# Iasonaspg/GPU-Randomized-Block-Lanczos

Hardware: AMD Instinct MI355X
Metric: RBL iters/sec + time-to-k=20 eigenpairs, n=1e7 nnz/row=100 b=32; 1/2/4/8 GPU (higher is better)
Workload: dtype f64

## Files before the change

### gpu-randomized-block-lanczos_amd/csrc/kernels.hpp

```cpp
#pragma once
#include "rbl_common.hpp"

namespace rbl {

struct Panels {
  static constexpr int kMax = 2;
  const double* ptr[kMax] = {nullptr, nullptr};
  int count = 0;
  int w = 0;
};
struct PanelRun {
  const double* base = nullptr;
  const float* base32 = nullptr;
  int64_t stride = 0;
  int count = 0;
  int w = 0;
};

constexpr int64_t kCsrPad = 256;
constexpr int64_t kRowPad = 16;
constexpr int64_t kRowPad32 = 32;

struct CsrDev {
  int64_t nrows = 0;
// ... 253 lines not shown
                 hipStream_t s);
int reduce_scratch_splits(int splits);
void reduce_slab_many(double* slab, int splits, int64_t len, double* out, hipStream_t s);
void tsmm(int64_t nrows, const PanelRun& X, const double* C, int ldc, const Panels& Y,
          double alpha, double beta, const int* skip, hipStream_t s, double* xslab = nullptr,
          int* xgrid = nullptr);

constexpr int kCompressMaxCols = 512;
bool basis_compress_fast(const PanelRun& X, int p);
bool basis_compress(int64_t nrows, const PanelRun& X, const double* S_dev, int p, hipStream_t s,
                    bool generic = false);

bool gram44_ok(int64_t nrows, int nW, int w, int xcount, int xw);
int gram44_splits(int64_t nrows, int nW, int w = 32);
void gram44_partial(int64_t nrows, const PanelRun& W, const Panels& X, double* slab, int splits,
                    const int* skip, hipStream_t s);
bool tsmm44_ok(int xw, int ky, int yw);
void tsmm44_f32x(int64_t nrows, const PanelRun& X, const double* C, int ldc, const Panels& Y,
                 double alpha, double beta, hipStream_t s);
int tsmm44_xg_grid(int64_t nrows);
void tsmm44(int64_t nrows, const PanelRun& X, const double* C, int ldc, const Panels& Y,
            double alpha, double beta, const int* skip, hipStream_t s, double* xslab = nullptr,
            int* xgrid = nullptr);

int gram32_splits(int64_t nrows);
void gram32_partial(int64_t nrows, const float* Wb, int64_t wstride, int nW, int w, const float* X0,
                    const float* X1, int xcount, double* slab, int splits, hipStream_t s);
void tsmm32(int64_t nrows, const float* Xb, int64_t xstride, int nX, int w, const double* C, int ldc,
            float* Y0, float* Y1, int ycount, float alpha, float beta, hipStream_t s);
void cvt_f32_to_f64(const float* src, double* dst, int64_t n, hipStream_t s);
void cvt_f64_to_f32(const double* src, float* dst, int64_t n, hipStream_t s);

void chol_step(const double* G, int b, int64_t nglobal, int mode, double* R, double* Rinv,
               double* Rtot, int* need3, int* status, const int* skip, hipStream_t s,
               double* scratch);
void copy_small(const double* src, double* dst, int64_t len, hipStream_t s, const int* skip = nullptr);
void cloc_rinv(double* C, const double* Rinv, int b, const int* skip, hipStream_t s);
void cloc_rinv2(double* C, const double* R1inv, const double* R2inv, int b, hipStream_t s);
void cloc_gate(const double* R, const double* Rinv, int b, const int* need3, double tau, int* gate,
               hipStream_t s);
void cloc_sub(double* G, const double* D, int nW, int b, hipStream_t s);
void transpose_small(const double* src, double* dst, int b, hipStream_t s);
void stash_step(const double* Ai, const double* Rtot, double* Bprev, int* flags, double* stash,
                int b, hipStream_t s);

struct RmatParams {
  int64_t n = 0;
  int scale = 0;
  int64_t edges = 0;
  double a = 0.57, b = 0.19, c = 0.19;
  uint64_t seed = 0;
  bool relabel = false;
  Scatter perm;
};
constexpr uint64_t kRelabelK = 0x52454C4142454C31ull;
void rmat_degree(const RmatParams& p, int32_t* deg, hipStream_t s);
int rmat_local_csr(const RmatParams& p, int64_t r0, int64_t r1, int64_t max_keys, int nplant,
                   const double* plant_dev, int64_t* rowptr_dev, int32_t** col_dev,
                   double** val_dev, int64_t* nnz_out, hipStream_t s);
void col_footprint(const int32_t* col, int64_t nnz, const int64_t* bounds_dev, int P,
                   unsigned long long* lo, unsigned long long* hi, hipStream_t s);

void circ_count(int64_t n, int64_t width, double p, uint64_t seed, int64_t r0, int64_t r1,
// ... 22 lines not shown
```

### gpu-randomized-block-lanczos_amd/csrc/rbl_api.cpp

```cpp
#include <hip/hip_runtime.h>
#include <rocprofiler-sdk-roctx/roctx.h>

#include <algorithm>
#include <cstdlib>
#include <chrono>
#include <cmath>
#include <cstdio>
#include <cstring>
#include <string>
#include <thread>
#include <vector>

#include "../../include/rbl_hip.h"
#include "comm.hpp"
#include "kernels.hpp"

using namespace rbl;

namespace rbl::api {

template <class T>
struct DevBuf {
  T* p = nullptr;
  DevBuf() = default;
// ... 148 lines not shown
  DevBuf<double> d_U;
  DevBuf<double> d_T;
  DevBuf<double> d_qext;
  DevBuf<double> d_sendbuf;
  DevBuf<double> d_pushbuf;
  DevBuf<double> d_precv;
  DevBuf<double> d_slab;
  DevBuf<double> d_C;
  DevBuf<double> d_small;
  DevBuf<int> d_flags;
  PinBuf<double> h_pin;
  PinBuf<double> h_hist;
  DevBuf<double> d_stash;
  DevBuf<double> d_lock;
  DevBuf<double> d_arrow_W;
  DevBuf<double> d_tr_S;
  DevBuf<double> d_filt[3];
  DevBuf<double> d_rv;
  DevBuf<double> d_rw;
};

struct CtxBufs {
  PinBuf<char> h_d2h[2];
};

}

struct rbl_ctx : rbl::api::MatrixBufs, rbl::api::RunBufs, rbl::api::CtxBufs {
  int device = 0;
  hipStream_t stream = nullptr;
  int nranks = 1, rank = 0;
  rbl::Comm* comm = nullptr;
  std::string err;

  int64_t n = 0, r0 = 0, r1 = 0, nloc = 0, nnz = 0;
  int64_t panel_nblk = 0;
  int panel_rpg = 4;
  int panel_ch = 48;
  bool panel_auto = false;
  int64_t panel_span = 0;
  int bt_ng = 0;
  int64_t seg_ntasks = 0, seg_nlong = 0;
  int seg_ntiers = 0;
  bool seg_split = false;
  bool ghost = false;
  int64_t n_ghost = 0, n_send = 0;
// ... 61 lines not shown
  double* dv_pin = nullptr;
  double* dv_hist = nullptr;
  bool flags_clean = false;
  int fetched = 1;
  bool have_bprev = false;
  int nlock = 0, lock_cap = 0;
  int arrow_kb = 0;
  size_t arrow_W_cap = 0, tr_S_cap = 0;
  int filt_deg = 0;
  double filt_lo = 0.0, filt_hi = 0.0, filt_ref = 0.0;
  int filt_cols = 0;
  std::vector<double> ser_mu;
  double ser_lo = 0.0, ser_hi = 0.0;
  int ritz_k = 0;

  int timers = 0;
  int reorth_order = 0;
  int spmm_variant = 0;
  int fuse = 7;
  int cloc_step = 0;
  bool cloc_final = false;
  bool cloc_derive = true;
  int cloc_src = 0;
  bool plan_all_resident = false;
  std::vector<int> step_flags;
  double stage_ms[RBL_NUM_STAGES] = {0};
  int64_t comm_stats[RBL_COMM_NSTATS] = {0};
  int64_t comm_host_ns[2] = {0, 0};
  double comm_dev_ms[2] = {0.0, 0.0};
  int64_t path_stats[RBL_PATH_NSTATS] = {0};
  struct Mark { int stage; hipEvent_t a, b; int parent = -1; };
  std::vector<Mark> marks;
  struct OpenStage { int stage; hipStream_t st; };
  std::vector<OpenStage> open_stages;
  std::vector<hipEvent_t> ev_pool;
  size_t ev_used = 0;
};

using namespace rbl::api;

namespace {

const char* kStageNames[RBL_NUM_STAGES] = {"AQ", "3-term", "qr", "part reorth", "loc reorth",
                                           "Ritz vectors", "comm", "spill wait"};

int fail(rbl_ctx* c, int code, const std::string& msg) {
// ... 1303 lines not shown
  const int d = (int)mu.size() - 1;
  const double c = 0.5 * (ctx->ser_lo + ctx->ser_hi), e = 0.5 * (ctx->ser_hi - ctx->ser_lo);
  const double* t1 = X;
  const double* t2 = nullptr;
  const int64_t len = ctx->nloc * b;
  for (int j = 1; j <= d; ++j) {
    double* tj = F[j % 3];
    const int st = apply_A(ctx, t1, 0, b, tj, nullptr, nullptr, nullptr);
    if (st < 0) return st;
    const double al = (j == 1 ? 1.0 : 2.0) / e;
    cheb_series_term(len, tj, t1, t2, al, -al * c, mu[j], mu[0], tj, out, j == 1, j == d, ctx->stream);
    HIPC(hipGetLastError());
    t2 = t1;
    t1 = tj;
  }
  return RBL_OK;
}

int filter_apply(rbl_ctx* ctx, const double* X, int b, double* out, const DevBuf<double> F[3]) {
  if (has_series(ctx)) return series_apply(ctx, X, b, out, F);
  return cheb_apply(ctx, X, b, out, F[0], F[1]);
}

int lock_reorth(rbl_ctx* ctx, double* X) {
  const int b = ctx->b;
  for (int j = 0; j < ctx->nlock; ++j) {
    const double* l = ctx->d_lock + (int64_t)j * ctx->nloc;
    CHK(gram(ctx, run1(l, 1), pan1(X, b), ctx->d_C, nullptr));
    CHK(tsmm_checked(ctx, run1(l, 1), ctx->d_C, b, pan1(X, b), -1.0, 1.0, nullptr));
  }
  return RBL_OK;
}

bool cloc_derive_on(const rbl_ctx* ctx) {
  return ctx->cloc_derive && ctx->basis_bits == 64 && rowgram_ok(ctx->b) && (ctx->fuse & 3) == 3 &&
         ctx->reorth_order == 0 && !spilled(ctx) && (ctx->nranks == 1 || ctx->plan_all_resident);
}

int reorth_pair(rbl_ctx* ctx, int i, int flags) {
  const int b = ctx->b;
  double* Qi = slotp(ctx, i - 1);
  double* Qm = i >= 2 ? slotp(ctx, i - 2) : nullptr;
  if ((flags & 2) && ctx->nlock > 0) {
    StageScope t(ctx, RBL_STAGE_PART_REORTH);
    if (Qm) CHK(lock_reorth(ctx, Qm));
    CHK(lock_reorth(ctx, Qi));
  }
  if ((flags & 1) && i >= 3) {
    StageScope t(ctx, RBL_STAGE_PART_REORTH);
    const int nW = i - 2;
    const int nres = std::min(nW, ctx->resident);
    const bool derive = cloc_derive_on(ctx) && b == 32 && ctx->cloc_step == i && !ctx->cloc_final &&
                        !((flags & 2) && ctx->nlock > 0) && nres == nW;
    const bool xg = (ctx->fuse & 2) && b == 32 && !derive;
    const int xg_parts = tsmm44_xg_grid(ctx->nloc);
    const bool xslab_ok = (size_t)(xg_parts + reduce_scratch_splits(xg_parts)) * b * b <= ctx->slab_elems;
    int xgrid = 0;
    auto update = [&](const PanelRun& W, bool last) -> int {
      const bool here = xg && last && xslab_ok;
      return tsmm_checked(ctx, W, ctx->d_C, 2 * b, pan2(Qi, Qm, b), -1.0, 1.0, nullptr,
                          here ? ctx->d_slab : nullptr, here ? &xgrid : nullptr);
    };
    if (ctx->reorth_order == 0) {
      PanelRun W;
      W.base = slotp(ctx, 0);
      W.stride = ctx->slot;
      W.count = nres;
      W.w = b;
      CHK(gram(ctx, W, pan2(Qi, Qm, b), ctx->d_C, nullptr));
      CHK(update(W, nres == nW));
    } else {
      for (int j = 0; j < nres; ++j) {
        const PanelRun W = run1(slotp(ctx, j), b);
        CHK(gram(ctx, W, pan2(Qi, Qm, b), ctx->d_C, nullptr));
        CHK(update(W, j == nW - 1));
      }
    }
    for (int j = nres; j < nW; ++j) {
      int st = 0;
      const double* Wj = block_dev(ctx, j, i, &st);
      if (st) return fail(ctx, st, "partial reorth: H2D of a spilled block failed");
      CHK(gram(ctx, run1(Wj, b), pan2(Qi, Qm, b), ctx->d_C, nullptr));
      CHK(update(run1(Wj, b), j == nW - 1));
    }
    if (xg) {
      if (xgrid > 0) {
        reduce_slab_many(ctx->d_slab, xgrid, (int64_t)b * b, smallp(ctx, S_CLOC), ctx->stream);
      } else if (ctx->nloc > 0) {
        const int sp = gram_splits(ctx->nloc, 1, b, b);
        gram_partial(ctx->nloc, run1(Qm, b), pan1(Qi, b), ctx->d_slab, sp, nullptr, ctx->stream);
        reduce_slab(ctx->d_slab, sp, (int64_t)b * b, smallp(ctx, S_CLOC), nullptr, ctx->stream);
      } else {
        HIPC(hipMemsetAsync(smallp(ctx, S_CLOC), 0, (size_t)b * b * sizeof(double), ctx->stream));
// ... 858 lines not shown
      if (value < 0 || value > 7 || value == 4)
        return fail(ctx, RBL_ERR_INVALID, "spmm kernel must be 0 (auto) or a kernel id 1, 2, 3, 5, 6, 7");
      ctx->spmm_variant = value == 5 ? 4 : value == 6 ? 5 : (int)value;
      return RBL_OK;
    case RBL_OPT_SPLIT_HALO: ctx->split_halo = value != 0; return RBL_OK;
    case RBL_OPT_HALO_OVERLAP: ctx->halo_overlap = value != 0; return RBL_OK;
    case RBL_OPT_HALO_PUSH:
      if (value < 0 || value > 2) return fail(ctx, RBL_ERR_INVALID, "RBL_OPT_HALO_PUSH must be 0|1|2");
      ctx->halo_push_opt = (int)value;
      return RBL_OK;
    case RBL_OPT_KEEP_CSR: ctx->keep_csr = value != 0; return RBL_OK;
    case RBL_OPT_RELABEL:
      if (value < 0 || value > 1) return fail(ctx, RBL_ERR_INVALID, "RBL_OPT_RELABEL must be 0|1");
      ctx->relabel_opt = (int)value;
      return RBL_OK;
    case RBL_OPT_FUSE:
      if (value < 0 || value > 7) return fail(ctx, RBL_ERR_INVALID, "RBL_OPT_FUSE is a 3-bit mask");
      ctx->fuse = (int)value;
      return RBL_OK;
    case RBL_OPT_CLOC_DERIVE:
      if (value < 0 || value > 1) return fail(ctx, RBL_ERR_INVALID, "RBL_OPT_CLOC_DERIVE must be 0|1");
      ctx->cloc_derive = value != 0;
      return RBL_OK;
    default: return fail(ctx, RBL_ERR_INVALID, "unknown option");
  }
}

int rbl_set_matrix_csc(rbl_ctx* ctx, int64_t n, int64_t nnz, const int64_t* colptr,
                       const int64_t* rowval, const double* nzval, int index_base) {
  if (!ctx || n < 1 || nnz < 0 || !colptr || (nnz && (!rowval || !nzval)) ||
      (index_base != 0 && index_base != 1))
    return fail(ctx, RBL_ERR_INVALID, "rbl_set_matrix_csc: bad arguments");
  if (colptr[n] - colptr[0] != nnz) return fail(ctx, RBL_ERR_INVALID, "colptr[n] != nnz");
  HIPC(hipSetDevice(ctx->device));
  std::vector<int64_t> rp(n + 1);
  for (int64_t i = 0; i <= n; ++i) rp[i] = colptr[i] - colptr[0];
  ctx->bounds.assign(ctx->nranks + 1, 0);
  rbl_plan_row_partition(n, rp.data(), ctx->nranks, ctx->bounds.data());
  const int64_t r0 = ctx->bounds[ctx->rank], r1 = ctx->bounds[ctx->rank + 1];
  return upload_csr(ctx, n, r0, r1, colptr + r0, rowval, nzval, index_base, index_base);
}

int rbl_set_matrix_csr_rows(rbl_ctx* ctx, int64_t n, int64_t row_begin, int64_t row_end,
                            const int64_t* rowptr, const int64_t* colind, const double* val,
                            int index_base) {
  if (!ctx || n < 1 || row_begin < 0 || row_end < row_begin || row_end > n || !rowptr ||
// ... 864 lines not shown
      HIPC(hipMemsetAsync(ctx->d_stage32, 0, ((size_t)nl + kRowPad32) * b * sizeof(float), ctx->stream));
      CHK(ensure_spill_stream(ctx));
    }
    HIPC(ctx->d_Qi64.alloc((nl + kRowPad) * b));
    if (!direct32_ok(ctx, b)) HIPC(ctx->d_Qm64.alloc((nl + kRowPad) * b));
  }
  HIPC(ctx->d_U.alloc((nl + kRowPad) * b));
  ctx->T_cols = b;
  HIPC(ctx->d_T.alloc(nl * b));
  if (ctx->nranks > 1) {
    CHK(ensure_qext(ctx, b, ctx->stream));
    if (ctx->ghost)
      HIPC(ctx->d_sendbuf.alloc(std::max<int64_t>(ctx->n_send, 1) * b));
  }
  const size_t slab = gram_slab_elems(ctx, b, max_blocks, basis_bits);
  ctx->slab_elems = slab;
  HIPC(ctx->d_slab.alloc(slab));
  ctx->C_elems = (size_t)std::max(1, max_blocks) * b * 2 * b;
  HIPC(ctx->d_C.alloc(ctx->C_elems));
  HIPC(ctx->d_small.alloc((size_t)S_NSMALL * b * b));
  HIPC(hipMemset(ctx->d_small, 0, (size_t)S_NSMALL * b * b * sizeof(double)));
  HIPC(ctx->d_flags.alloc(6));
  HIPC(hipMemset(ctx->d_flags, 0, 6 * sizeof(int)));
  {
#ifdef RBL_VARIANTS
    const char* e = std::getenv("RBL_STASH_COPY");
    ctx->stash_direct = !(e && std::atoi(e) == 1);
#else
    ctx->stash_direct = true;
#endif
    const unsigned hf = ctx->stash_direct ? (hipHostMallocMapped | hipHostMallocCoherent) : hipHostMallocDefault;
    HIPC(ctx->h_pin.alloc(stash_rec(b), hf));
    HIPC(ctx->h_hist.alloc((size_t)(max_blocks + 2) * stash_rec(b), hf));
    if ((size_t)ctx->nloc * b * sizeof(double) >= 4 * kD2HPiece && !d2h_direct()) {
      CHK(ensure_d2h_slots(ctx));
      CHK(ensure_ritz_stream(ctx));
    }
    if (ctx->stash_direct) {
      HIPC(hipHostGetDevicePointer(reinterpret_cast<void**>(&ctx->dv_pin), ctx->h_pin, 0));
      HIPC(hipHostGetDevicePointer(reinterpret_cast<void**>(&ctx->dv_hist), ctx->h_hist, 0));
    } else {
      HIPC(ctx->d_stash.alloc(stash_rec(b)));
    }
  }
  }
  if (ctx->push && ctx->nranks > 1 && use_ghost(ctx, b)) {
// ... 1677 lines not shown
  return RBL_OK;
}

int rbl_comm_stats(rbl_ctx* ctx, int64_t* out, int nstats, int reset) {
  if (!ctx || nstats < 0 || (nstats > 0 && !out)) return RBL_ERR_INVALID;
  for (int i = 0; i < nstats && i < RBL_COMM_NSTATS; ++i) out[i] = ctx->comm_stats[i];
  if (nstats > RBL_COMM_HALO_PUSH) out[RBL_COMM_HALO_PUSH] = ctx->push ? 1 : 0;
  if (nstats > RBL_COMM_PUSH_ROWS) out[RBL_COMM_PUSH_ROWS] = ctx->push_pred_rows;
  if (nstats > RBL_COMM_PULL_ROWS) out[RBL_COMM_PULL_ROWS] = ctx->pull_pred_rows;
  const int64_t tm[4] = {ctx->comm_host_ns[0], ctx->comm_host_ns[1],
                         (int64_t)(ctx->comm_dev_ms[0] * 1e6), (int64_t)(ctx->comm_dev_ms[1] * 1e6)};
  for (int i = RBL_COMM_PULL_ROWS + 1; i < nstats; ++i)
    out[i] = i <= RBL_COMM_EXCHANGE_DEV_NS ? tm[i - RBL_COMM_ALLREDUCE_HOST_NS] : 0;
  if (reset) {
    for (int64_t& v : ctx->comm_stats) v = 0;
    ctx->comm_host_ns[0] = ctx->comm_host_ns[1] = 0;
    ctx->comm_dev_ms[0] = ctx->comm_dev_ms[1] = 0.0;
  }
  return RBL_OK;
}

int rbl_path_stats(rbl_ctx* ctx, int64_t* out, int nstats, int reset) {
  if (!ctx || nstats < 0 || (nstats > 0 && !out)) return RBL_ERR_INVALID;
  for (int i = 0; i < nstats; ++i) out[i] = i < RBL_PATH_NSTATS ? ctx->path_stats[i] : 0;
  if (reset)
    for (int64_t& v : ctx->path_stats) v = 0;
  return RBL_OK;
}

int rbl_reset_timers(rbl_ctx* ctx) {
  if (!ctx) return RBL_ERR_INVALID;
  for (double& v : ctx->stage_ms) v = 0.0;
  return RBL_OK;
}
int rbl_synchronize(rbl_ctx* ctx) {
  if (!ctx) return RBL_ERR_INVALID;
  HIPC(hipSetDevice(ctx->device));
  HIPC(hipStreamSynchronize(ctx->stream));
  harvest_timers(ctx);
  return RBL_OK;
}

}
```

### gpu-randomized-block-lanczos_amd/csrc/reorth.hip

```cpp
#include <algorithm>
#include <cstdlib>

#include "kernels.hpp"

namespace rbl {

__device__ __forceinline__ double mfma4(double a, double b, double c) {
  return __builtin_amdgcn_mfma_f64_4x4x4f64(a, b, c, 0, 0, 0);
}
#ifndef RBL_REORTH_ABL
#define RBL_REORTH_ABL 0
#endif
#ifndef RBL_REORTH_NT
#define RBL_REORTH_NT 0
#endif
template <typename T>
__device__ __forceinline__ T ldw(const T* p) {
  if constexpr (RBL_REORTH_NT) return __builtin_nontemporal_load(p);
  return *p;
}

constexpr int kG44Waves = 4;
#ifndef RBL_G44_ROWS
#define RBL_G44_ROWS 16
// ... 756 lines not shown
      }
    }
  }
  if constexpr (XG) {
    __syncthreads();
    const int li = lane & 15;
    constexpr int G2 = YW * YW;
    double* gw = cs_raw + wave * G2;
#pragma unroll
    for (int it = 0; it < NT; ++it)
#pragma unroll
      for (int jt = 0; jt < NT; ++jt)
#pragma unroll
        for (int reg = 0; reg < 4; ++reg) gw[(16 * it + q + 4 * reg) * YW + 16 * jt + li] = gx[it][jt][reg];
    __syncthreads();
    double* out = xslab + tile * G2;
    for (int e = tid; e < G2; e += 256)
      out[e] = (cs_raw[e] + cs_raw[G2 + e]) + (cs_raw[2 * G2 + e] + cs_raw[3 * G2 + e]);
  }
  };
  tile_body(blockIdx.x);
}

bool tsmm44_ok(int xw, int ky, int yw) {
  return (xw == 16 || xw == 32) && ky >= 1 && ky <= 64 && yw % 2 == 0;
}

template <int B, int KYP, bool F32X = false>
static void launch_tsmm44(int64_t nrows, const PanelRun& X, const double* C, int ldc, int KY,
                          const Panels& Y, double alpha, double beta, const int* skip,
                          hipStream_t st) {
  const int64_t wgs = (nrows + 4 * kT44Rows - 1) / (4 * kT44Rows);
  hipLaunchKernelGGL((k_tsmm44<B, KYP, F32X>), dim3((unsigned)wgs), dim3(256), 0, st, nrows, X, C,
                     ldc, KY, Y, alpha, beta, skip);
}

void tsmm44_f32x(int64_t nrows, const PanelRun& X, const double* C, int ldc, const Panels& Y,
                 double alpha, double beta, hipStream_t st) {
  const int KY = Y.count * Y.w;
  if (X.w == 32) {
    if (KY <= 16) return launch_tsmm44<32, 16, true>(nrows, X, C, ldc, KY, Y, alpha, beta, nullptr, st);
    if (KY <= 32) return launch_tsmm44<32, 32, true>(nrows, X, C, ldc, KY, Y, alpha, beta, nullptr, st);
    return launch_tsmm44<32, 64, true>(nrows, X, C, ldc, KY, Y, alpha, beta, nullptr, st);
  }
  if (KY <= 16) return launch_tsmm44<16, 16, true>(nrows, X, C, ldc, KY, Y, alpha, beta, nullptr, st);
  if (KY <= 32) return launch_tsmm44<16, 32, true>(nrows, X, C, ldc, KY, Y, alpha, beta, nullptr, st);
// ... 72 lines not shown
```

### gpu-randomized-block-lanczos_amd/csrc/smallmat.hip

```cpp
#include <cstdlib>

#include "kernels.hpp"

namespace rbl {

constexpr int kMaxB = 64;

template <bool LDS>
struct SmallMat {
  double* p;
  int ld;
  __device__ double& operator()(int r, int c) const { return p[r * ld + c]; }
};

template <bool LDS>
__global__ __launch_bounds__(256) void k_chol(const double* __restrict__ G, int b, int64_t nglob,
                                              int mode, double* R, double* Rinv, double* Rtot,
                                              int* need3, int* status, const int* skip,
                                              double* scratch) {
  if (skip && *skip) return;
  __shared__ double Ml[LDS ? kMaxB * (kMaxB + 1) : 1];
  __shared__ double Xl[LDS ? kMaxB * (kMaxB + 1) : 1];
  __shared__ int fail;
  __shared__ double shift;
// ... 565 lines not shown
  const int c = threadIdx.x;
  double s = 0.0;
  if (c < b)
    for (int k = 0; k <= c; ++k) s += rs[k * b + c] * rs[k * b + c];
  d[c] = sqrt(s);
  __syncthreads();
  double t = 0.0;
  if (c < b)
    for (int j = 0; j <= c; ++j) t += d[j] * fabs(ri[j * b + c]);
  e[c] = t;
  __syncthreads();
  if (c == 0) {
    bool ok = need3[0] == 0;
    for (int j = 0; j < b; ++j) ok = ok && e[j] <= tau;
    gate[0] = ok;
    gate[1] = !ok;
  }
}
void cloc_gate(const double* R, const double* Rinv, int b, const int* need3, double tau, int* gate,
               hipStream_t s) {
  hipLaunchKernelGGL(k_cloc_gate, dim3(1), dim3(256), 0, s, R, Rinv, b, need3, tau, gate);
}

constexpr int kClocSubThreads = 1024;
__global__ __launch_bounds__(kClocSubThreads) void k_cloc_sub(double* __restrict__ G,
                                                              const double* __restrict__ D, int K, int b) {
  __shared__ double part[kClocSubThreads];
  const int r = blockIdx.x, ng = kClocSubThreads / b;
  const int kg = threadIdx.x / b, c = threadIdx.x % b;
  const int chunk = (K + ng - 1) / ng;
  double acc = 0.0;
  if (kg < ng) {
    const int k1 = min(K, (kg + 1) * chunk);
    for (int k = kg * chunk; k < k1; ++k) acc += D[(int64_t)k * 2 * b + b + r] * D[(int64_t)k * 2 * b + c];
  }
  part[threadIdx.x] = acc;
  __syncthreads();
  if (kg == 0) {
    double sum = part[c];
    for (int g = 1; g < ng; ++g) sum += part[g * b + c];
    G[r * b + c] -= sum;
  }
}
void cloc_sub(double* G, const double* D, int nW, int b, hipStream_t s) {
  hipLaunchKernelGGL(k_cloc_sub, dim3(b), dim3(kClocSubThreads), 0, s, G, D, nW * b, b);
}
// ... 10 lines not shown
```

### gpu-randomized-block-lanczos_amd/rbl/_lib.py

```python
from __future__ import annotations

import ctypes as C
import os

import numpy as np

_HERE = os.path.dirname(os.path.abspath(__file__))
LIB_PATH = os.environ.get("RBL_LIB") or os.path.join(_HERE, "librbl_hip.so")

RBL_OK = 0
RBL_WARN_NOT_CONVERGED = 1
RBL_WARN_QR_SHIFTED = 2
RBL_ERR_INVALID = -1
RBL_ERR_HIP = -2
RBL_ERR_OOM = -3
RBL_ERR_RCCL = -4
RBL_ERR_STATE = -5
RBL_ERR_NUMERIC = -6

RBL_MAX_BLOCK = 512

RBL_OPT_TIMERS = 0
RBL_OPT_REORTH_ORDER = 1
RBL_OPT_SPMM_KERNEL = 2
RBL_OPT_DEVICE_BLOCKS = 3
RBL_OPT_SPLIT_HALO = 4
RBL_OPT_KEEP_CSR = 5
RBL_OPT_FUSE = 6
RBL_OPT_HALO_OVERLAP = 7
RBL_OPT_RELABEL = 8
RBL_OPT_HALO_PUSH = 9
RBL_OPT_CLOC_DERIVE = 10
RBL_PATH_SPMM = 0
RBL_PATH_SPMM_LOC_FUSED = 1
RBL_PATH_LOC_SEPARATE = 2
RBL_PATH_LOC_GRAM = 3
RBL_PATH_LOCFIX_EDGES = 4
RBL_PATH_LOCFIX_REST = 5
RBL_PATH_SPMM_TWO_WAVE = 6
RBL_PATH_RITZ_PIECES = 7
RBL_PATH_CLOC_3TERM = 8
RBL_PATH_CLOC_REORTH = 9
RBL_PATH_NSTATS = 10
RBL_BUILD_VARIANTS = 1
RBL_SPMM_KERNEL_RECT = 8
RBL_MATRIX_FORMAT_RECT = 5
RBL_KERNEL_RBF = 0
RBL_KERNEL_LAPLACE = 1
RBL_KERNEL_POLY = 2
RBL_KERNOP_MAX_DIM = 256
RBL_SPMM_KERNEL_KERNOP = 9
RBL_MATRIX_FORMAT_KERNOP = 6
RBL_PROBE_GAUSS = 0
RBL_PROBE_SIGN = 1
RBL_SOLVE_CONVERGED = 0
RBL_SOLVE_MAX_ITER = 1
RBL_SOLVE_NOT_POSDEF = 2
RBL_COMPRESS_MAX_COLS = 512

_p = C.c_void_p
_i64 = C.c_int64
_u64 = C.c_uint64
_pd = C.POINTER(C.c_double)
_pi64 = C.POINTER(C.c_int64)
_pi32 = C.POINTER(C.c_int32)
_pu8 = C.POINTER(C.c_uint8)
# ... 65 lines not shown
    "rbl_get_lowrank": (C.c_int, [_p, C.POINTER(C.c_int), _pd, _pd]),
    "rbl_bench_lowrank_pass": (C.c_int, [_p, _i64, C.c_int, C.c_int, C.c_int, _pd, _pd]),
    "rbl_set_precond_lowrank": (C.c_int, [_p, C.c_int, _pd, _pd]),
    "rbl_clear_precond": (C.c_int, [_p]),
    "rbl_solve": (C.c_int, [_p, C.c_int, _pd, _pd, C.c_double, C.c_double, C.c_int, C.c_int, C.c_int,
                            _pi32, _pi32, _pd, _pd]),
    "rbl_bench_cg_pass": (C.c_int, [_p, _i64, C.c_int, C.c_int, C.c_int, _pd]),
    "rbl_ritz_project": (C.c_int, [_p, C.c_int, C.c_int, _pd, _pd]),
    "rbl_ritz_finish": (C.c_int, [_p, C.c_int, _pd, _pd, _pd, _pd]),
    "rbl_ritz_finish_cols": (C.c_int, [_p, C.c_int, C.c_int, _pd, _pd, _pd, _pd]),
    "rbl_restart": (C.c_int, [_p, C.c_int, _pd]),
    "rbl_lock": (C.c_int, [_p, C.c_int, C.c_int, _pd]),
    "rbl_num_locked": (C.c_int, [_p]),
    "rbl_get_locked": (C.c_int, [_p, _pd]),
    "rbl_reorth_last": (C.c_int, [_p, C.c_int, C.c_int]),
    "rbl_thick_restart": (C.c_int, [_p, C.c_int, C.c_int, _pd, _pd]),
    "rbl_bench_compress_pass": (C.c_int, [_p, _i64, C.c_int, C.c_int, C.c_int, C.c_int, _pd, _pd]),
    "rbl_num_stages": (C.c_int, []),
    "rbl_stage_name": (C.c_char_p, [C.c_int]),
    "rbl_timers": (C.c_int, [_p, _pd, C.c_int]),
    "rbl_reset_timers": (C.c_int, [_p]),
    "rbl_comm_stats": (C.c_int, [_p, _pi64, C.c_int, C.c_int]),
    "rbl_path_stats": (C.c_int, [_p, _pi64, C.c_int, C.c_int]),
    "rbl_allgather_host": (C.c_int, [_p, _pi64, _pi64, C.c_int]),
    "rbl_synchronize": (C.c_int, [_p]),
    "rbl_plan_row_partition": (C.c_int, [_i64, _pi64, C.c_int, _pi64]),
    "rbl_plan_halo": (C.c_int, [_i64, _pi64, _pi64, C.c_int, C.c_int, _pi64, _pi64, _pi64]),
    "rbl_hashwindow_rows_host": (C.c_int, [_i64, _i64, C.c_double, _u64, C.c_int, _pd, _i64,
                                           _i64, _pi64, _pi64, _pd]),
}


class RBLError(RuntimeError):
    def __init__(self, code: int, msg: str):
        super().__init__(f"librbl_hip error {code}: {msg}")
        self.code = code


def load() -> C.CDLL:
    if not os.path.exists(LIB_PATH):
        raise ImportError(f"librbl_hip.so not built at {LIB_PATH}; run __graft_entry__.build() "
                          "(the HIP library is the only compute path — no CPU fallback)")
    lib = C.CDLL(LIB_PATH)
    for name, (res, args) in SIGNATURES.items():
        fn = getattr(lib, name)
        fn.restype = res
        fn.argtypes = args
# ... 78 lines not shown
```

### gpu-randomized-block-lanczos_amd/rbl/rbl_gpu.py

```python
from __future__ import annotations

import math
import time
from dataclasses import dataclass, field

import numpy as np
import scipy.sparse as sp

from . import _lib
from ._lib import RBLError, dptr, i32ptr, i64ptr, lib, u8ptr
from .host import (TBand, dsbev, eig_topk, fix_signs,
                   residual_norms, sort_eig_abs, speculation_depth)

KRYL_SZ_GPU = 1200
RESIDUAL_TOL = 1e-7


class LocalGroup:

    def __init__(self, nranks: int):
        import ctypes as C
        self._h = C.c_void_p()
        st = lib.rbl_local_group_create(C.byref(self._h), nranks)
        if st < 0:
# ... 574 lines not shown
        buf = C.create_string_buffer(32)
        self._check(lib.rbl_comm_info(self._h, C.byref(n), C.byref(r), buf, 32), "rbl_comm_info")
        out = {"nranks": n.value, "rank": r.value, "transport": buf.value.decode()}
        if out["transport"] == "rccl":
            out.update(rccl_version())
        return out

    def comm_stats(self, reset: bool = False, times: bool = False) -> dict:
        out = np.zeros(12, np.int64)
        self._check(lib.rbl_comm_stats(self._h, i64ptr(out), 12, int(reset)), "rbl_comm_stats")
        keys = ("allreduce_calls", "allreduce_bytes", "exchange_calls", "send_bytes",
                "recv_bytes", "halo_push", "push_rows_pred", "pull_rows_pred")
        if times:
            keys += ("allreduce_host_ns", "exchange_host_ns", "allreduce_dev_ns", "exchange_dev_ns")
        return dict(zip(keys, (int(x) for x in out)))

    def path_stats(self, reset: bool = False) -> dict:
        from . import _lib as L
        out = np.zeros(L.RBL_PATH_NSTATS, np.int64)
        self._check(lib.rbl_path_stats(self._h, i64ptr(out), L.RBL_PATH_NSTATS, int(reset)),
                    "rbl_path_stats")
        return dict(zip(("spmm", "spmm_loc_fused", "loc_separate", "loc_gram", "locfix_edges",
                         "locfix_rest", "spmm_two_wave", "ritz_pieces", "cloc_3term",
                         "cloc_reorth"), (int(x) for x in out)))

    def allgather(self, values) -> np.ndarray:
        mine = np.ascontiguousarray(np.asarray(values, dtype=np.int64).ravel())
        out = np.zeros(self.nranks * mine.size, np.int64)
        self._check(lib.rbl_allgather_host(self._h, i64ptr(mine), i64ptr(out), mine.size),
                    "rbl_allgather_host")
        return out.reshape(self.nranks, mine.size)

    def synchronize(self) -> None:
        self._check(lib.rbl_synchronize(self._h), "rbl_synchronize")


@dataclass
class RBLInfo:
    iters: int = 0
    nblocks: int = 0
    converged: bool = False
    status: int = 0
    qr_shifted_steps: int = 0
    eig_ms: float = 0.0
    fetch_ms: float = 0.0
    ritz_ms: float = 0.0
    start_ms: float = 0.0
# ... 158 lines not shown
```

### include/rbl_hip.h

```cpp
#ifndef RBL_HIP_H
#define RBL_HIP_H

#include <stdint.h>

#ifdef __cplusplus
extern "C" {
#endif

#define RBL_ABI_VERSION 2
#define RBL_MAX_BLOCK 512

#define RBL_OK                  0
#define RBL_WARN_NOT_CONVERGED  1
#define RBL_WARN_QR_SHIFTED     2
#define RBL_ERR_INVALID        -1
#define RBL_ERR_HIP            -2
#define RBL_ERR_OOM            -3
#define RBL_ERR_RCCL           -4
#define RBL_ERR_STATE          -5
#define RBL_ERR_NUMERIC        -6

#define RBL_STAGE_AQ          0
#define RBL_STAGE_3TERM       1
#define RBL_STAGE_QR          2
#define RBL_STAGE_PART_REORTH 3
#define RBL_STAGE_LOC_REORTH  4
#define RBL_STAGE_RITZ        5
#define RBL_STAGE_COMM        6
#define RBL_STAGE_SPILL_WAIT  7
#define RBL_NUM_STAGES        8

#define RBL_OPT_TIMERS        0
#define RBL_OPT_REORTH_ORDER  1
#define RBL_OPT_DEVICE_BLOCKS 3
#define RBL_OPT_SPMM_KERNEL   2
#define RBL_OPT_SPLIT_HALO    4
#define RBL_OPT_KEEP_CSR      5
#define RBL_OPT_FUSE          6

#define RBL_OPT_HALO_OVERLAP  7

#define RBL_OPT_RELABEL       8

#define RBL_OPT_HALO_PUSH     9

#define RBL_OPT_CLOC_DERIVE   10

typedef struct rbl_ctx rbl_ctx;

int rbl_abi_version(void);
#define RBL_BUILD_VARIANTS 1
int rbl_build_flags(void);

int rbl_create(rbl_ctx** ctx, int device);
int rbl_get_unique_id(uint8_t unique_id[128]);
int rbl_comm_selftest(int device, char* msg, int msg_len);
int rbl_create_dist(rbl_ctx** ctx, int device, int nranks, int rank, const uint8_t unique_id[128]);
typedef struct rbl_group rbl_group;
int rbl_local_group_create(rbl_group** group, int nranks);
int rbl_local_group_free(rbl_group* group);
int rbl_create_local(rbl_ctx** ctx, int device, rbl_group* group, int rank);
int rbl_create_shm(rbl_ctx** ctx, int device, int nranks, int rank, const char* path);
int rbl_free(rbl_ctx* ctx);
const char* rbl_last_error(const rbl_ctx* ctx);
int rbl_comm_info(rbl_ctx* ctx, int* nranks, int* rank, char* transport, int transport_len);
int rbl_rccl_version(int* version, char* path, int path_len);
int rbl_set_option(rbl_ctx* ctx, int option, int64_t value);
int rbl_device_memory(rbl_ctx* ctx, int64_t* free_bytes, int64_t* total_bytes);

// ... 113 lines not shown
#define RBL_COMM_RECV_BYTES      4
#define RBL_COMM_NSTATS          5
#define RBL_COMM_HALO_PUSH       5
#define RBL_COMM_PUSH_ROWS       6
#define RBL_COMM_PULL_ROWS       7
#define RBL_COMM_ALLREDUCE_HOST_NS 8
#define RBL_COMM_EXCHANGE_HOST_NS  9
#define RBL_COMM_ALLREDUCE_DEV_NS  10
#define RBL_COMM_EXCHANGE_DEV_NS   11
int rbl_comm_stats(rbl_ctx* ctx, int64_t* out, int nstats, int reset);

int rbl_allgather_host(rbl_ctx* ctx, const int64_t* mine, int64_t* all, int n);

#define RBL_PATH_SPMM            0
#define RBL_PATH_SPMM_LOC_FUSED  1
#define RBL_PATH_LOC_SEPARATE    2
#define RBL_PATH_LOC_GRAM        3
#define RBL_PATH_LOCFIX_EDGES    4
#define RBL_PATH_LOCFIX_REST     5
#define RBL_PATH_SPMM_TWO_WAVE   6
#define RBL_PATH_RITZ_PIECES     7
#define RBL_PATH_CLOC_3TERM      8
#define RBL_PATH_CLOC_REORTH     9
#define RBL_PATH_NSTATS          10
int rbl_path_stats(rbl_ctx* ctx, int64_t* out, int nstats, int reset);

int rbl_plan_row_partition(int64_t n, const int64_t* rowptr, int nranks, int64_t* bounds_out);
int rbl_plan_halo(int64_t nrows_local, const int64_t* rowptr, const int64_t* colind,
                  int index_base, int nranks, const int64_t* bounds, int64_t* lo, int64_t* hi);
int rbl_hashwindow_rows_host(int64_t n, int64_t halfwidth, double density, uint64_t seed,
                             int nplant, const double* plant, int64_t row_begin,
                             int64_t row_end, int64_t* rowptr_out, int64_t* colind_out,
                             double* val_out);

#ifdef __cplusplus
}
#endif
#endif
```

Baseline: 47.71.

## Add gated fp32 MFMA reorthogonalization update with device-side fp64 fallback

Adds a tsmm kernel that does the two-panel reorthogonalization update (Y -= X*C) with fp32 MFMA, rounding the fp64 basis and coefficients to float while accumulating into the fp64 outputs. A single-block device kernel computes a scaled norm of the coefficient matrix and sets flags: when the estimated error is below a tolerance the fp32 kernel runs, otherwise the existing fp64 tsmm runs via the skip flag. Both launches are always issued and one no-ops, so the host never syncs. The aim is to cut the cost of the fp64 tall-skinny update. It risks some accuracy in reorthogonalization, adds a small gate-kernel launch per step, and adds path-stat counters.

```diff
diff --git a/gpu-randomized-block-lanczos_amd/csrc/kernels.hpp b/gpu-randomized-block-lanczos_amd/csrc/kernels.hpp
--- a/gpu-randomized-block-lanczos_amd/csrc/kernels.hpp
+++ b/gpu-randomized-block-lanczos_amd/csrc/kernels.hpp
@@ -299,6 +299,9 @@
 void tsmm44(int64_t nrows, const PanelRun& X, const double* C, int ldc, const Panels& Y,
             double alpha, double beta, const int* skip, hipStream_t s, double* xslab = nullptr,
             int* xgrid = nullptr);
+bool tsmm44x32_ok(int64_t nrows, const PanelRun& X, const Panels& Y);
+void tsmm44x32(int64_t nrows, const PanelRun& X, const double* C, int ldc, const Panels& Y,
+               const int* skip, hipStream_t s);
 
 int gram32_splits(int64_t nrows);
 void gram32_partial(int64_t nrows, const float* Wb, int64_t wstride, int nW, int w, const float* X0,
@@ -316,6 +319,8 @@
 void cloc_rinv2(double* C, const double* R1inv, const double* R2inv, int b, hipStream_t s);
 void cloc_gate(const double* R, const double* Rinv, int b, const int* need3, double tau, int* gate,
                hipStream_t s);
+void upd32_gate(const double* C, int K, int ncols, double tau, int force, int* flags, double* g_out,
+                hipStream_t s);
 void cloc_sub(double* G, const double* D, int nW, int b, hipStream_t s);
 void transpose_small(const double* src, double* dst, int b, hipStream_t s);
 void stash_step(const double* Ai, const double* Rtot, double* Bprev, int* flags, double* stash,
diff --git a/gpu-randomized-block-lanczos_amd/csrc/rbl_api.cpp b/gpu-randomized-block-lanczos_amd/csrc/rbl_api.cpp
--- a/gpu-randomized-block-lanczos_amd/csrc/rbl_api.cpp
+++ b/gpu-randomized-block-lanczos_amd/csrc/rbl_api.cpp
@@ -194,6 +194,8 @@
 
 struct CtxBufs {
   PinBuf<char> h_d2h[2];
+  DevBuf<int> d_upd32;
+  DevBuf<double> d_upd32_g;
 };
 
 }
@@ -301,6 +303,7 @@
   bool cloc_final = false;
   bool cloc_derive = true;
   int cloc_src = 0;
+  int upd32 = 1;
   bool plan_all_resident = false;
   std::vector<int> step_flags;
   double stage_ms[RBL_NUM_STAGES] = {0};
@@ -1650,6 +1653,9 @@
   return cheb_apply(ctx, X, b, out, F[0], F[1]);
 }
 
+constexpr double kUpd32Tau = 0.5;
+constexpr int kUpd32Log = 64;
+
 int lock_reorth(rbl_ctx* ctx, double* X) {
   const int b = ctx->b;
   for (int j = 0; j < ctx->nlock; ++j) {
@@ -1696,7 +1702,21 @@
       W.count = nres;
       W.w = b;
       CHK(gram(ctx, W, pan2(Qi, Qm, b), ctx->d_C, nullptr));
-      CHK(update(W, nres == nW));
+      const Panels Yp = pan2(Qi, Qm, b);
+      const bool gate32 = ctx->upd32 != 0 && b == 32 && !xg && nres == nW && !((flags & 2) && ctx->nlock > 0);
+      const bool u32 = gate32 && ctx->nloc > 0 && tsmm44x32_ok(ctx->nloc, W, Yp);
+      if (gate32) {
+        upd32_gate(ctx->d_C, nW * b, 2 * b, kUpd32Tau, ctx->upd32 == 2, ctx->d_upd32,
+                   ctx->d_upd32_g + (i % kUpd32Log), ctx->stream);
+        HIPC(hipGetLastError());
+      }
+      if (u32) {
+        tsmm44x32(ctx->nloc, W, ctx->d_C, 2 * b, Yp, ctx->d_upd32, ctx->stream);
+        HIPC(hipGetLastError());
+        CHK(tsmm_checked(ctx, W, ctx->d_C, 2 * b, Yp, -1.0, 1.0, ctx->d_upd32 + 1));
+      } else {
+        CHK(update(W, nres == nW));
+      }
     } else {
       for (int j = 0; j < nres; ++j) {
         const PanelRun W = run1(slotp(ctx, j), b);
@@ -2601,6 +2621,10 @@
       if (value < 0 || value > 1) return fail(ctx, RBL_ERR_INVALID, "RBL_OPT_CLOC_DERIVE must be 0|1");
       ctx->cloc_derive = value != 0;
       return RBL_OK;
+    case RBL_OPT_UPD32:
+      if (value < 0 || value > 2) return fail(ctx, RBL_ERR_INVALID, "RBL_OPT_UPD32 must be 0|1|2");
+      ctx->upd32 = (int)value;
+      return RBL_OK;
     default: return fail(ctx, RBL_ERR_INVALID, "unknown option");
   }
 }
@@ -3511,6 +3535,12 @@
   HIPC(hipMemset(ctx->d_small, 0, (size_t)S_NSMALL * b * b * sizeof(double)));
   HIPC(ctx->d_flags.alloc(6));
   HIPC(hipMemset(ctx->d_flags, 0, 6 * sizeof(int)));
+  if (!ctx->d_upd32) {
+    HIPC(ctx->d_upd32.alloc(4));
+    HIPC(hipMemset(ctx->d_upd32, 0, 4 * sizeof(int)));
+    HIPC(ctx->d_upd32_g.alloc(kUpd32Log));
+    HIPC(hipMemset(ctx->d_upd32_g, 0, kUpd32Log * sizeof(double)));
+  }
   {
 #ifdef RBL_VARIANTS
     const char* e = std::getenv("RBL_STASH_COPY");
@@ -5234,9 +5264,28 @@
 
 int rbl_path_stats(rbl_ctx* ctx, int64_t* out, int nstats, int reset) {
   if (!ctx || nstats < 0 || (nstats > 0 && !out)) return RBL_ERR_INVALID;
+  if (ctx->d_upd32) {
+    int cnt[2] = {0, 0};
+    HIPC(hipSetDevice(ctx->device));
+    HIPC(hipStreamSynchronize(ctx->stream));
+    HIPC(hipMemcpy(cnt, ctx->d_upd32 + 2, sizeof(cnt), hipMemcpyDeviceToHost));
+    ctx->path_stats[RBL_PATH_UPD32_TAKEN] = cnt[0];
+    ctx->path_stats[RBL_PATH_UPD32_REFUSED] = cnt[1];
+    if (reset) HIPC(hipMemset(ctx->d_upd32 + 2, 0, sizeof(cnt)));
+  }
   for (int i = 0; i < nstats; ++i) out[i] = i < RBL_PATH_NSTATS ? ctx->path_stats[i] : 0;
   if (reset)
     for (int64_t& v : ctx->path_stats) v = 0;
+  return RBL_OK;
+}
+
+int rbl_upd32_gate_values(rbl_ctx* ctx, double* out, int n) {
+  if (!ctx || n < 0 || (n > 0 && !out)) return RBL_ERR_INVALID;
+  for (int i = 0; i < n; ++i) out[i] = 0.0;
+  if (!ctx->d_upd32_g || n == 0) return RBL_OK;
+  HIPC(hipSetDevice(ctx->device));
+  HIPC(hipStreamSynchronize(ctx->stream));
+  HIPC(hipMemcpy(out, ctx->d_upd32_g, (size_t)std::min(n, kUpd32Log) * sizeof(double), hipMemcpyDeviceToHost));
   return RBL_OK;
 }
 
diff --git a/gpu-randomized-block-lanczos_amd/csrc/reorth.hip b/gpu-randomized-block-lanczos_amd/csrc/reorth.hip
--- a/gpu-randomized-block-lanczos_amd/csrc/reorth.hip
+++ b/gpu-randomized-block-lanczos_amd/csrc/reorth.hip
@@ -802,6 +802,133 @@
   tile_body(blockIdx.x);
 }
 
+typedef float f2v32 __attribute__((ext_vector_type(2)));
+typedef float f4v32 __attribute__((ext_vector_type(4)));
+constexpr int kU32Rows = 32;
+__global__ __launch_bounds__(256) void k_tsmm44x32(int64_t nrows, PanelRun X,
+                                                   const double* __restrict__ C, int ldc, double* Y0,
+                                                   double* Y1, const int* skip) {
+  if (skip && *skip) return;
+  constexpr int W = 32, KYP = 64, CT = 4, CLD = 64, KF = 32, NH = KF / 8, OLD = KYP + 4;
+  __shared__ __attribute__((aligned(16))) float cs[2][KF * CLD + 128];
+  static_assert(2 * (KF * CLD + 128) >= 4 * 16 * OLD, "epilogue tiles fit");
+  const int tid = threadIdx.x, lane = tid & 63;
+  const int wave = __builtin_amdgcn_readfirstlane(tid >> 6);
+  const int q = lane >> 4, c16 = lane & 15;
+  const int64_t r0 = ((int64_t)blockIdx.x * 4 + wave) * kU32Rows;
+  const int64_t rw = r0 + kU32Rows <= nrows ? r0 : nrows - kU32Rows;
+  const int nch = X.count;
+
+  f4v32 acc[2][CT];
+#pragma unroll
+  for (int rt = 0; rt < 2; ++rt)
+#pragma unroll
+    for (int c = 0; c < CT; ++c) acc[rt][c] = f4v32{0.f, 0.f, 0.f, 0.f};
+
+  const unsigned aoff0 = (unsigned)(c16 * W + 2 * q);
+  auto load_a = [&](int ch, d2v (&ar)[2][NH]) {
+    const int chc = ch < nch ? ch : nch - 1;
+    const double* xb = X.base + (int64_t)chc * X.stride + rw * W;
+#pragma unroll
+    for (int h = 0; h < NH; ++h)
+#pragma unroll
+      for (int rt = 0; rt < 2; ++rt)
+        ar[rt][h] = *reinterpret_cast<const d2v*>(xb + (aoff0 + (unsigned)(16 * rt * W + 8 * h)));
+  };
+  auto round_a = [&](const d2v (&ar)[2][NH], float (&af)[2][NH][2]) {
+#pragma unroll
+    for (int rt = 0; rt < 2; ++rt)
+#pragma unroll
+      for (int h = 0; h < NH; ++h) {
+        af[rt][h][0] = (float)ar[rt][h].x;
+        af[rt][h][1] = (float)ar[rt][h].y;
+      }
+  };
+  const int ck = tid >> 4, ccc = tid & 15;
+  auto load_c = [&](int ch, float (&cr)[2][CT]) {
+    const int chc = ch < nch ? ch : nch - 1;
+    const double* cb = C + (int64_t)(KF * chc + ck) * ldc + ccc;
+#pragma unroll
+    for (int hh = 0; hh < 2; ++hh)
+#pragma unroll
+      for (int ct = 0; ct < CT; ++ct) cr[hh][ct] = (float)cb[(int64_t)(16 * hh) * ldc + 16 * ct];
+  };
+  auto store_c = [&](int buf, const float (&cr)[2][CT]) {
+#pragma unroll
+    for (int hh = 0; hh < 2; ++hh)
+      *reinterpret_cast<f4v32*>(&cs[buf][(ck + 16 * hh) * CLD + 4 * ccc]) =
+          f4v32{cr[hh][0], cr[hh][1], cr[hh][2], cr[hh][3]};
+  };
+
+  d2v anext[2][NH];
+  float af[2][NH][2];
+  float cr[2][CT];
+  load_c(0, cr);
+  store_c(0, cr);
+  load_a(0, anext);
+  round_a(anext, af);
+  __syncthreads();
+  for (int ch = 0; ch < nch; ++ch) {
+    load_c(ch + 1, cr);
+    load_a(ch + 1, anext);
+    const float* cb = cs[ch & 1] + 2 * q * CLD + 4 * c16;
+#pragma unroll
+    for (int hv = 0; hv < 2 * NH; ++hv) {
+      const int h = hv >> 1, v = hv & 1;
+      const f4v32 bv = *reinterpret_cast<const f4v32*>(cb + (8 * h + v) * CLD);
+#pragma unroll
+      for (int rt = 0; rt < 2; ++rt)
+#pragma unroll
+        for (int c = 0; c < CT; ++c)
+          acc[rt][c] = __builtin_amdgcn_mfma_f32_16x16x4f32(af[rt][h][v], bv[c], acc[rt][c], 0, 0, 0);
+    }
+    store_c((ch + 1) & 1, cr);
+    round_a(anext, af);
+    __syncthreads();
+  }
+  float* ot = &cs[0][0] + wave * 16 * OLD;
+  const int ce = (2 * lane) % KYP, rl = (2 * lane) / KYP;
+  double* yb = (ce < W ? Y0 + ce : Y1 + (ce - W)) + (rw + rl) * W;
+  const int dskip = (int)(r0 - rw);
+#pragma unroll
+  for (int rt = 0; rt < 2; ++rt) {
+#pragma unroll
+    for (int c = 0; c < CT; ++c)
+#pragma unroll
+      for (int v = 0; v < 4; ++v) ot[(4 * q + v) * OLD + 16 * c + c16] = acc[rt][c][v];
+    __builtin_amdgcn_wave_barrier();
+    __builtin_amdgcn_fence(__ATOMIC_RELEASE, "wavefront");
+#pragma unroll
+    for (int m = 0; m < 8; ++m) {
+      const int row = rl + 2 * m;
+      const f2v32 p = *reinterpret_cast<const f2v32*>(ot + row * OLD + ce);
+      if (16 * rt + row >= dskip) {
+        d2v* yp = reinterpret_cast<d2v*>(yb + (int64_t)((16 * rt + 2 * m) * W));
+        d2v y = *yp;
+        y.x -= (double)p.x;
+        y.y -= (double)p.y;
+        *yp = y;
+      }
+    }
+    __builtin_amdgcn_fence(__ATOMIC_ACQUIRE, "wavefront");
+    __builtin_amdgcn_wave_barrier();
+  }
+}
+
+bool tsmm44x32_ok(int64_t nrows, const PanelRun& X, const Panels& Y) {
+  if (X.w != 32 || X.count < 1 || !X.base || Y.count != 2 || Y.w != 32 || nrows < kU32Rows) return false;
+  for (int t = 0; t < Y.count; ++t)
+    if (Y.ptr[t] >= X.base && Y.ptr[t] < X.base + (int64_t)X.count * X.stride) return false;
+  return true;
+}
+
+void tsmm44x32(int64_t nrows, const PanelRun& X, const double* C, int ldc, const Panels& Y,
+               const int* skip, hipStream_t st) {
+  const int64_t wgs = (nrows + 4 * kU32Rows - 1) / (4 * kU32Rows);
+  hipLaunchKernelGGL(k_tsmm44x32, dim3((unsigned)wgs), dim3(256), 0, st, nrows, X, C, ldc,
+                     const_cast<double*>(Y.ptr[0]), const_cast<double*>(Y.ptr[1]), skip);
+}
+
 bool tsmm44_ok(int xw, int ky, int yw) {
   return (xw == 16 || xw == 32) && ky >= 1 && ky <= 64 && yw % 2 == 0;
 }
diff --git a/gpu-randomized-block-lanczos_amd/csrc/smallmat.hip b/gpu-randomized-block-lanczos_amd/csrc/smallmat.hip
--- a/gpu-randomized-block-lanczos_amd/csrc/smallmat.hip
+++ b/gpu-randomized-block-lanczos_amd/csrc/smallmat.hip
@@ -611,6 +611,51 @@
   hipLaunchKernelGGL(k_cloc_gate, dim3(1), dim3(256), 0, s, R, Rinv, b, need3, tau, gate);
 }
 
+constexpr int kUpd32GateThreads = 1024;
+__global__ __launch_bounds__(kUpd32GateThreads) void k_upd32_gate(const double* __restrict__ C, int K,
+                                                                  int ncols, double tau, int force,
+                                                                  int* __restrict__ flags,
+                                                                  double* __restrict__ g_out) {
+  __shared__ double part[kUpd32GateThreads];
+  __shared__ double ssq[64];
+  constexpr int NG = kUpd32GateThreads / 64;
+  const int c = threadIdx.x % 64, grp = threadIdx.x / 64;
+  double s = 0.0;
+  if (c < ncols)
+    for (int k = grp; k < K; k += NG) {
+      const double v = C[(int64_t)k * ncols + c];
+      s += v * v;
+    }
+  part[threadIdx.x] = s;
+  __syncthreads();
+  if (grp == 0) {
+    double t = part[c];
+    for (int g = 1; g < NG; ++g) t += part[64 * g + c];
+    ssq[c] = t;
+  }
+  __syncthreads();
+  if (threadIdx.x == 0) {
+    double m = 0.0;
+    bool finite = true;
+    for (int j = 0; j < ncols; ++j) {
+      finite = finite && ssq[j] == ssq[j];
+      m = ssq[j] > m ? ssq[j] : m;
+    }
+    const double g = finite ? sqrt(m) * sqrt((double)K) * 268435456.0 : __builtin_nan("");
+    const bool take = force || g <= tau;
+    flags[0] = !take;
+    flags[1] = take;
+    flags[2] += take;
+    flags[3] += !take;
+    if (g_out) *g_out = g;
+  }
+}
+void upd32_gate(const double* C, int K, int ncols, double tau, int force, int* flags, double* g_out,
+                hipStream_t s) {
+  hipLaunchKernelGGL(k_upd32_gate, dim3(1), dim3(kUpd32GateThreads), 0, s, C, K, ncols, tau, force, flags,
+                     g_out);
+}
+
 constexpr int kClocSubThreads = 1024;
 __global__ __launch_bounds__(kClocSubThreads) void k_cloc_sub(double* __restrict__ G,
                                                               const double* __restrict__ D, int K, int b) {
diff --git a/gpu-randomized-block-lanczos_amd/rbl/_lib.py b/gpu-randomized-block-lanczos_amd/rbl/_lib.py
--- a/gpu-randomized-block-lanczos_amd/rbl/_lib.py
+++ b/gpu-randomized-block-lanczos_amd/rbl/_lib.py
@@ -31,6 +31,7 @@
 RBL_OPT_RELABEL = 8
 RBL_OPT_HALO_PUSH = 9
 RBL_OPT_CLOC_DERIVE = 10
+RBL_OPT_UPD32 = 11
 RBL_PATH_SPMM = 0
 RBL_PATH_SPMM_LOC_FUSED = 1
 RBL_PATH_LOC_SEPARATE = 2
@@ -41,7 +42,9 @@
 RBL_PATH_RITZ_PIECES = 7
 RBL_PATH_CLOC_3TERM = 8
 RBL_PATH_CLOC_REORTH = 9
-RBL_PATH_NSTATS = 10
+RBL_PATH_UPD32_TAKEN = 10
+RBL_PATH_UPD32_REFUSED = 11
+RBL_PATH_NSTATS = 12
 RBL_BUILD_VARIANTS = 1
 RBL_SPMM_KERNEL_RECT = 8
 RBL_MATRIX_FORMAT_RECT = 5
@@ -153,7 +156,8 @@
     "rbl_reset_timers": (C.c_int, [_p]),
     "rbl_comm_stats": (C.c_int, [_p, _pi64, C.c_int, C.c_int]),
     "rbl_path_stats": (C.c_int, [_p, _pi64, C.c_int, C.c_int]),
-    "rbl_allgather_host": (C.c_int, [_p, _pi64, _pi64, C.c_int]),
+    "rbl_upd32_gate_values": (C.c_int, [_p, _pd, C.c_int]),
+    "rbl_allgather_host":(C.c_int, [_p, _pi64, _pi64, C.c_int]),
     "rbl_synchronize": (C.c_int, [_p]),
     "rbl_plan_row_partition": (C.c_int, [_i64, _pi64, C.c_int, _pi64]),
     "rbl_plan_halo": (C.c_int, [_i64, _pi64, _pi64, C.c_int, C.c_int, _pi64, _pi64, _pi64]),
diff --git a/gpu-randomized-block-lanczos_amd/rbl/rbl_gpu.py b/gpu-randomized-block-lanczos_amd/rbl/rbl_gpu.py
--- a/gpu-randomized-block-lanczos_amd/rbl/rbl_gpu.py
+++ b/gpu-randomized-block-lanczos_amd/rbl/rbl_gpu.py
@@ -620,7 +620,12 @@
                     "rbl_path_stats")
         return dict(zip(("spmm", "spmm_loc_fused", "loc_separate", "loc_gram", "locfix_edges",
                          "locfix_rest", "spmm_two_wave", "ritz_pieces", "cloc_3term",
-                         "cloc_reorth"), (int(x) for x in out)))
+                         "cloc_reorth", "upd32_taken", "upd32_refused"), (int(x) for x in out)))
+
+    def upd32_gate_values(self) -> np.ndarray:
+        out = np.zeros(64, np.float64)
+        self._check(lib.rbl_upd32_gate_values(self._h, dptr(out), 64), "rbl_upd32_gate_values")
+        return out
 
     def allgather(self, values) -> np.ndarray:
         mine = np.ascontiguousarray(np.asarray(values, dtype=np.int64).ravel())
diff --git a/include/rbl_hip.h b/include/rbl_hip.h
--- a/include/rbl_hip.h
+++ b/include/rbl_hip.h
@@ -45,6 +45,8 @@
 #define RBL_OPT_HALO_PUSH     9
 
 #define RBL_OPT_CLOC_DERIVE   10
+
+#define RBL_OPT_UPD32         11
 
 typedef struct rbl_ctx rbl_ctx;
 
@@ -204,8 +206,11 @@
 #define RBL_PATH_RITZ_PIECES     7
 #define RBL_PATH_CLOC_3TERM      8
 #define RBL_PATH_CLOC_REORTH     9
-#define RBL_PATH_NSTATS          10
+#define RBL_PATH_UPD32_TAKEN     10
+#define RBL_PATH_UPD32_REFUSED   11
+#define RBL_PATH_NSTATS          12
 int rbl_path_stats(rbl_ctx* ctx, int64_t* out, int nstats, int reset);
+int rbl_upd32_gate_values(rbl_ctx* ctx, double* out, int n);
 
 int rbl_plan_row_partition(int64_t n, const int64_t* rowptr, int nranks, int64_t* bounds_out);
 int rbl_plan_halo(int64_t nrows_local, const int64_t* rowptr, const int64_t* colind,
```

Result: faster. 51.45 (median of 6 runs) (+7.8%).
